# swesterfeld/audiowmark

Hardware: NVIDIA B200
Metric: audio frames/sec embed+detect, 44.1 kHz stereo; decoded-bit match vs ref (higher is better)
Workload: dtype f32

## Files before the change

audiowmark_b200/csrc/awm_capi.cu:

```cuda
#include "awm_kernels.cuh"
#include "awm_speed.cuh"
#include "awm_refine_slide.cuh"
#include "awm_approx_mags.cuh"
#include <vector>
#include <time.h>
#include <string.h>
#include "awm_approx_tc.cuh"
#include "awm_embed_strip.cuh"
#include "awm_viterbi_pair.cuh"

#include <cuda_runtime.h>
#include <dlfcn.h>
#include <algorithm>
#include <map>
#include <thread>
#include <limits.h>
#include <math.h>
#include <stdarg.h>
#include <stdio.h>
#include <string.h>
#include <string>
#include <vector>

using namespace awm;
// ... 49 lines not shown
          }
        if (cur + 1 < chunks.size())
          {
            cur++;
            off = 0;
            continue;
          }
        Chunk c { nullptr, std::max<size_t> (n, size_t (4) << 20) };
        if (cudaMallocHost (reinterpret_cast<void **> (&c.p), c.cap) != cudaSuccess)
          return nullptr;
        chunks.push_back (c);
        cur = chunks.size() - 1;
        off = 0;
      }
  }
  template<class T> T *get (size_t count) { return static_cast<T *> (alloc (std::max<size_t> (count, 1) * sizeof (T))); }
  void release()
  {
    for (auto& c : chunks)
      cudaFreeHost (c.p);
    chunks.clear();
    reset();
  }
};

inline double
wall_now()
{
  timespec ts;
  clock_gettime (CLOCK_MONOTONIC, &ts);
  return double (ts.tv_sec) + 1e-9 * double (ts.tv_nsec);
}

struct SyncTab
{
  DevBuf ent, off, sorted, groups;
  DevBuf masks, masks48, masks64;
  int n_chunks = 0, n_chunks48 = 0, n_chunks64 = 0;
  int n_groups = 0;
  int n_ent = 0, n_bits = 0, total_frames = 0;
  std::vector<awm_sync_entry> h_ent;
  std::vector<int> h_off;
};

struct KeyTab
{
  SyncTab sync[2];
  DevBuf mix, order;
  int n_mix = 0, n_coded = 0, frames_per_bit = 0, fpb = 0;
};

}

struct awm_ctx
{
  int device = 0;
  cudaStream_t stream = nullptr;
  cudaStream_t s_in = nullptr, s_out = nullptr;
  std::string err;
  uint64_t launches = 0;
  int n_sms = 0;
  bool profiling = false;
  struct ProfRec { const char *name; cudaEvent_t e0, e1; double bytes; };
  std::vector<ProfRec> prof;

  DevBuf tw, win, synth;
  DevBuf frame_mod; int embed_fpb = 0;
  KeyTab keys[AWM_MAX_KEYS];

  const float *pcm = nullptr; size_t pcm_frames = 0; int pcm_ch = 0;
  DevBuf pcm_own, pcm16_own;
  struct Prefetch { DevBuf buf, buf16; bool s16 = false; const void *src = nullptr; size_t n_frames = 0; int ch = 0; cudaEvent_t done = nullptr; bool valid = false; };
  Prefetch pref[2];
  int pref_next = 0;
  DevBuf staged, staged16;
  std::vector<cudaEvent_t> stage_done;
  size_t stage_piece = 0, stage_frames = 0, stage_converted = 0;
  int stage_ch = 0;
  bool stage_s16 = false;

  DevBuf dbT, have, q, scores, a_ud, a_cnt, peaks_out, peaks_cnt, a_mags;
  size_t n_scores_dev = 0;
  DevBuf cand_start, cand_noff, r_ud, r_cnt, rvalid, r_ent_ud, r_ent_flag, tw1024;
  DevBuf blk_start, D, raw;
  DevBuf vit_raw, vit_off, vit_types, vit_delta, vit_dec, vit_bits, vit_err, vit_order;
  DevBuf emb_in, emb_out, emb_in16, emb_out16, peaks, snr;

  PinArena pin;

  void *nccl_comm = nullptr;
  int dist_rank = 0, dist_world = 1;
  DevBuf dist_send, dist_recv;
  unsigned char *dist_hsend = nullptr, *dist_hhdr = nullptr;
  size_t dist_hsend_cap = 0;

  struct CoefTab { DevBuf buf; int h = 0; };
  std::map<std::pair<double, int>, CoefTab> coef_cache;
  DevBuf rs_in, rs_out, rs_jobs, pcm_rs;
  const float *saved_pcm = nullptr; size_t saved_frames = 0; int saved_ch = 0; bool pushed = false;
  DevBuf win512, sp_clip, sp_sub, sp_mags, sp_mag_jobs, sp_cmp_jobs, sp_best;
};

namespace {

int
fail (awm_ctx *ctx, const char *fmt, ...)
{
  char buf[512];
  va_list ap;
  va_start (ap, fmt);
  vsnprintf (buf, sizeof (buf), fmt, ap);
  va_end (ap);
  if (ctx)
    ctx->err = buf;
  return 1;
}

#define CK(call) do { cudaError_t e_ = (call); if (e_ != cudaSuccess) return fail (ctx, "%s: %s", #call, cudaGetErrorString (e_)); } while (0)
#define LAUNCH_CHECK(name) do { ctx->launches++; cudaError_t e_ = cudaGetLastError(); if (e_ != cudaSuccess) return fail (ctx, "launch %s: %s", name, cudaGetErrorString (e_)); prof_end (ctx, name); } while (0)
#define PROF(ctx) prof_begin (ctx)

void
prof_begin (awm_ctx *ctx)
{
  if (!ctx->profiling)
    return;
  awm_ctx::ProfRec r;
  r.name = nullptr;
  r.bytes = 0;
  cudaEventCreate (&r.e0);
  cudaEventCreate (&r.e1);
  cudaEventRecord (r.e0, ctx->stream);
  ctx->prof.push_back (r);
}

void
prof_end (awm_ctx *ctx, const char *name)
{
  if (!ctx->profiling || ctx->prof.empty() || ctx->prof.back().name)
    return;
  ctx->prof.back().name = name;
  cudaEventRecord (ctx->prof.back().e1, ctx->stream);
}

void
prof_bytes (awm_ctx *ctx, double bytes)
{
  if (ctx->profiling && !ctx->prof.empty())
    ctx->prof.back().bytes = bytes;
}

bool
is_device_ptr (const void *p)
{
  cudaPointerAttributes a;
  if (cudaPointerGetAttributes (&a, p) != cudaSuccess)
    {
      cudaGetLastError();
      return false;
    }
  return a.type == cudaMemoryTypeDevice || a.type == cudaMemoryTypeManaged;
}

double
window_cos (double x)
{
// ... 21 lines not shown
      weight += w;
    }
  for (int i = 0; i < kFrame; i++)
    win[i] *= 2.0 / weight;
  std::vector<float> synth (3 * kFrame);
  for (int i = 0; i < 3 * kFrame; i++)
    {
      const double overlap = 0.1;
      double norm_pos = (double (i) - kFrame) / kFrame;
      if (norm_pos > 0.5)
        norm_pos = 1 - norm_pos;
      double tri;
      if (norm_pos < -overlap)
        tri = 0;
      else if (norm_pos < overlap)
        tri = 0.5 + norm_pos / (2 * overlap);
      else
        tri = 1;
      synth[i] = (cos (tri * M_PI + M_PI) + 1) * 0.5;
    }
  CK (ctx->tw.reserve (tw.size() * sizeof (float2)));
  CK (ctx->win.reserve (win.size() * sizeof (float)));
  CK (ctx->synth.reserve (synth.size() * sizeof (float)));
  CK (cudaMemcpy (ctx->tw.p, tw.data(), tw.size() * sizeof (float2), cudaMemcpyHostToDevice));
  CK (cudaMemcpy (ctx->win.p, win.data(), win.size() * sizeof (float), cudaMemcpyHostToDevice));
  CK (cudaMemcpy (ctx->synth.p, synth.data(), synth.size() * sizeof (float), cudaMemcpyHostToDevice));
  return 0;
}

template<class K> int
set_smem (awm_ctx *ctx, K kernel, size_t bytes)
{
  static std::map<std::pair<const void *, int>, size_t> done;
  size_t& have = done[{ reinterpret_cast<const void *> (kernel), ctx->device }];
  if (have >= bytes && have)
    return 0;
  CK (cudaFuncSetAttribute (kernel, cudaFuncAttributeMaxDynamicSharedMemorySize, int (bytes)));
  have = bytes;
  return 0;
}

}

void nccl_destroy (void *comm);

extern "C" {

int
awm_create (int device, awm_ctx **out)
{
  if (!out)
    return 1;
  *out = nullptr;
  int n_dev = 0;
  if (cudaGetDeviceCount (&n_dev) != cudaSuccess || n_dev <= 0)
    return 2;
  if (device < 0 || device >= n_dev)
    return 3;
  awm_ctx *ctx = new awm_ctx();
  ctx->device = device;
  if (cudaSetDevice (device) != cudaSuccess || cudaStreamCreateWithFlags (&ctx->stream, cudaStreamNonBlocking) != cudaSuccess)
    {
      delete ctx;
      return 4;
    }
  if (init_tables (ctx))
    {
      fprintf (stderr, "awm_create: %s\n", ctx->err.c_str());
      delete ctx;
      return 5;
    }
  *out = ctx;
  return 0;
}

void
awm_destroy (awm_ctx *ctx)
{
  if (!ctx)
    return;
  cudaSetDevice (ctx->device);
  cudaStreamSynchronize (ctx->stream);
  DevBuf *bufs[] = { &ctx->tw, &ctx->win, &ctx->synth, &ctx->frame_mod, &ctx->pcm_own, &ctx->pcm16_own, &ctx->dbT, &ctx->have, &ctx->q, &ctx->scores, &ctx->a_ud, &ctx->a_cnt, &ctx->peaks_out, &ctx->peaks_cnt, &ctx->a_mags,
                     &ctx->cand_start, &ctx->cand_noff, &ctx->r_ud, &ctx->r_cnt, &ctx->rvalid, &ctx->r_ent_ud, &ctx->r_ent_flag, &ctx->tw1024, &ctx->vit_off, &ctx->blk_start, &ctx->D, &ctx->raw,
                     &ctx->vit_raw, &ctx->vit_types, &ctx->vit_delta, &ctx->vit_dec, &ctx->vit_bits, &ctx->vit_err, &ctx->vit_order,
                     &ctx->emb_in, &ctx->emb_out, &ctx->emb_in16, &ctx->emb_out16, &ctx->peaks, &ctx->snr, &ctx->rs_in, &ctx->rs_out, &ctx->rs_jobs, &ctx->pcm_rs,
                     &ctx->win512, &ctx->sp_clip, &ctx->sp_sub, &ctx->sp_mags, &ctx->sp_mag_jobs, &ctx->sp_cmp_jobs, &ctx->sp_best };
  for (DevBuf *b : bufs)
    b->release();
  ctx->pin.release();
  ctx->dist_send.release();
  ctx->dist_recv.release();
  if (ctx->dist_hsend) cudaFreeHost (ctx->dist_hsend);
  if (ctx->dist_hhdr) cudaFreeHost (ctx->dist_hhdr);
  if (ctx->nccl_comm)
    nccl_destroy (ctx->nccl_comm);
  for (auto& ct : ctx->coef_cache)
    ct.second.buf.release();
  for (auto& pf : ctx->pref)
    {
      pf.buf.release();
      pf.buf16.release();
      if (pf.done)
        cudaEventDestroy (pf.done);
    }
  for (KeyTab& k : ctx->keys)
    {
      for (SyncTab& s : k.sync)
        {
          s.ent.release();
          s.masks.release();
          s.masks48.release();
          s.masks64.release();
          s.off.release();
          s.sorted.release();
          s.groups.release();
        }
      k.mix.release();
      k.order.release();
    }
  for (cudaEvent_t e : ctx->stage_done)
    cudaEventDestroy (e);
  if (ctx->s_in)
    cudaStreamDestroy (ctx->s_in);
  if (ctx->s_out)
    cudaStreamDestroy (ctx->s_out);
  cudaStreamDestroy (ctx->stream);
  delete ctx;
}

const char *
awm_last_error (const awm_ctx *ctx)
{
  return ctx ? ctx->err.c_str() : "no context (is a CUDA device present? there is no CPU fallback)";
}

uint64_t
awm_launch_count (const awm_ctx *ctx)
{
  return ctx ? ctx->launches : 0;
}

void *
awm_stream (awm_ctx *ctx)
{
  return ctx ? (void *) ctx->stream : nullptr;
}

int
awm_synchronize (awm_ctx *ctx)
{
  CK (cudaSetDevice (ctx->device));
  CK (cudaStreamSynchronize (ctx->stream));
  return 0;
}

void *
awm_host_alloc (size_t bytes)
{
  void *p = nullptr;
  if (cudaHostAlloc (&p, bytes ? bytes : 1, cudaHostAllocDefault) != cudaSuccess)
    {
      cudaGetLastError();
      return nullptr;
    }
  return p;
}
// ... 955 lines not shown
  CK (cudaSetDevice (ctx->device));
  const int total = fpb * (mode == AWM_MODE_CLIP ? 2 : 1);
  const double norm_div = water_delta < 0.080 ? water_delta : 0.080;

  const size_t nc = n_scores;
  const int n_bits = t.n_bits;
  CK (ctx->cand_start.reserve (nc * sizeof (long long)));
  CK (ctx->cand_noff.reserve (nc * sizeof (int)));
  CK (ctx->r_ud.reserve (nc * kOffsets * n_bits * 2 * sizeof (float)));
  CK (ctx->r_cnt.reserve (nc * kOffsets * n_bits * sizeof (int)));
  CK (ctx->rvalid.reserve (nc * kOffsets));
  ctx->pin.reset();
  long long *h_start = ctx->pin.get<long long> (nc);
  int *h_noff = ctx->pin.get<int> (nc);
  if (!h_start || !h_noff)
    return fail (ctx, "awm_sync_refine: out of page-locked memory");
  for (size_t c = 0; c < nc; c++)
    {
      const long long idx = (long long) scores[c].index;
      const long long start = std::max<long long> (idx - 256, 0), end = idx + 256;
      h_start[c] = start;
      h_noff[c] = int (std::min<long long> ((end - start) / 8 + 1, kOffsets));
    }
  CK (cudaMemcpyAsync (ctx->cand_start.p, h_start, nc * sizeof (long long), cudaMemcpyHostToDevice, ctx->stream));
  CK (cudaMemcpyAsync (ctx->cand_noff.p, h_noff, nc * sizeof (int), cudaMemcpyHostToDevice, ctx->stream));
  static const bool force_fft = [] { const char *e = getenv ("AWM_REFINE"); return e && !strcmp (e, "fft"); } ();
  const bool used_slide = force < 0 ? (ctx->pcm_ch <= 2 && !force_fft) : (force == 0 && ctx->pcm_ch <= 2);
  if (used_slide)
    {
      if (!ctx->tw1024.p)
        {
          std::vector<float2> tw (1024);
          for (int p = 0; p < 1024; p++)
            {
              const double a = -2.0 * M_PI * double (p) / 1024.0;
              tw[p] = make_float2 (float (cos (a)), float (sin (a)));
            }
          CK (ctx->tw1024.reserve (tw.size() * sizeof (float2)));
          CK (cudaMemcpy (ctx->tw1024.p, tw.data(), tw.size() * sizeof (float2), cudaMemcpyHostToDevice));
        }
      const size_t n_pairs = size_t (nc) * kOffsets * t.n_ent;
      CK (ctx->r_ent_ud.reserve (n_pairs * sizeof (float2)));
      CK (ctx->r_ent_flag.reserve (n_pairs));
      const size_t smem = fft_smem_bytes (kSlideWarps);
      const long long jobs = (long long) nc * t.n_ent;
      const unsigned grid = unsigned ((jobs + kSlideWarps - 1) / kSlideWarps);
      PROF (ctx);
      if (ctx->pcm_ch == 2)
        {
          if (set_smem (ctx, k_refine_slide<2>, smem)) return 1;
          k_refine_slide<2><<<grid, kSlideWarps * 32, smem, ctx->stream>>> (ctx->pcm, (long long) ctx->pcm_frames, ctx->cand_start.as<long long>(), ctx->cand_noff.as<int>(), int (nc),
            t.ent.as<awm_sync_entry>(), t.n_ent, total, (long long) wav_first, (long long) wav_last, ctx->r_ent_ud.as<float2>(), ctx->r_ent_flag.as<unsigned char>(),
            ctx->tw.as<float2>(), ctx->tw1024.as<float2>());
        }
      else
        {
          if (set_smem (ctx, k_refine_slide<1>, smem)) return 1;
          k_refine_slide<1><<<grid, kSlideWarps * 32, smem, ctx->stream>>> (ctx->pcm, (long long) ctx->pcm_frames, ctx->cand_start.as<long long>(), ctx->cand_noff.as<int>(), int (nc),
            t.ent.as<awm_sync_entry>(), t.n_ent, total, (long long) wav_first, (long long) wav_last, ctx->r_ent_ud.as<float2>(), ctx->r_ent_flag.as<unsigned char>(),
            ctx->tw.as<float2>(), ctx->tw1024.as<float2>());
        }
      LAUNCH_CHECK ("k_refine_slide");
      prof_bytes (ctx, double (nc) * double (t.n_ent) * (double (kFrame) + 512.0) * ctx->pcm_ch * sizeof (float));
      const long long n_red = (long long) nc * kOffsets * n_bits;
      PROF (ctx);
      k_refine_reduce<<<unsigned ((n_red + 127) / 128), 128, 0, ctx->stream>>> (ctx->r_ent_ud.as<float2>(), ctx->r_ent_flag.as<unsigned char>(), int (nc), t.n_ent,
        t.off.as<int>(), n_bits, ctx->cand_start.as<long long>(), ctx->cand_noff.as<int>(), (long long) ctx->pcm_frames, total,
        ctx->r_ud.as<float>(), ctx->r_cnt.as<int>(), ctx->rvalid.as<unsigned char>());
      LAUNCH_CHECK ("k_refine_reduce");
    }
  else
    {
      const size_t smem = fft_smem_bytes (kRefineWarps) + kRefineWarps * 96 * sizeof (float);
      if (set_smem (ctx, k_refine, smem)) return 1;
      const long long jobs = (long long) nc * kOffsets * n_bits;
      PROF (ctx);
      k_refine<<<unsigned ((jobs + kRefineWarps - 1) / kRefineWarps), kRefineWarps * 32, smem, ctx->stream>>> (
        ctx->pcm, (long long) ctx->pcm_frames, ctx->pcm_ch, ctx->cand_start.as<long long>(), ctx->cand_noff.as<int>(), int (nc),
        t.ent.as<awm_sync_entry>(), t.off.as<int>(), n_bits, total, (long long) wav_first, (long long) wav_last,
        ctx->r_ud.as<float>(), ctx->r_cnt.as<int>(), ctx->rvalid.as<unsigned char>(), ctx->tw.as<float2>(), ctx->win.as<float>());
      LAUNCH_CHECK ("k_refine");
      prof_bytes (ctx, double (nc) * double (t.n_ent) * (double (kFrame) + 512.0) * ctx->pcm_ch * sizeof (float));
    }
  const size_t n_ud = nc * kOffsets * n_bits * 2, n_cnt = nc * kOffsets * n_bits, n_val = nc * kOffsets;
  float *h_ud = ctx->pin.get<float> (n_ud);
  int *h_cnt = ctx->pin.get<int> (n_cnt);
  unsigned char *h_valid = ctx->pin.get<unsigned char> (n_val);
  if (!h_ud || !h_cnt || !h_valid)
    return fail (ctx, "awm_sync_refine: out of page-locked memory");
  CK (cudaMemcpyAsync (h_ud, ctx->r_ud.p, n_ud * sizeof (float), cudaMemcpyDeviceToHost, ctx->stream));
  CK (cudaMemcpyAsync (h_cnt, ctx->r_cnt.p, n_cnt * sizeof (int), cudaMemcpyDeviceToHost, ctx->stream));
  CK (cudaMemcpyAsync (h_valid, ctx->rvalid.p, n_val, cudaMemcpyDeviceToHost, ctx->stream));
  CK (cudaStreamSynchronize (ctx->stream));
  auto quality_of = [&] (const float *ud, const int *cnt, size_t base) -> double
    {
      double sync_quality = 0;
      int bit_count = 0;
      for (int bit = 0; bit < n_bits; bit++)
        {
          const size_t ob = base * n_bits + bit;
          const float umag = ud[ob * 2], dmag = ud[ob * 2 + 1];
          double raw_bit;
          if (umag == 0 || dmag == 0)
            raw_bit = 0;
          else if (umag < dmag)
            raw_bit = 1 - umag / dmag;
          else
            raw_bit = dmag / umag - 1;
          sync_quality += ((bit & 1) ? raw_bit : -raw_bit) * cnt[ob];
          bit_count += cnt[ob];
        }
      if (bit_count)
        sync_quality /= bit_count;
      return sync_quality / norm_div / 2.9;
    };
  if (q_out)
    {
      for (size_t c = 0; c < nc; c++)
        for (int o = 0; o < kOffsets; o++)
          {
            const bool v = o < h_noff[c] && h_valid[c * kOffsets + o];
            valid_out[c * kOffsets + o] = v ? 1 : 0;
            q_out[c * kOffsets + o] = v ? quality_of (h_ud, h_cnt, c * kOffsets + o) : 0.0;
          }
      return 0;
    }
  if (used_slide)
    {
      constexpr double kVerifyMargin = 1e-3;
      std::vector<long long> p_start;
      std::vector<int> p_noff, p_cand, p_off;
      for (size_t c = 0; c < nc; c++)
        {
          std::vector<std::pair<double, int>> ranked;
          for (int o = 0; o < h_noff[c]; o++)
            if (h_valid[c * kOffsets + o])
              ranked.push_back ({ -fabs (quality_of (h_ud, h_cnt, c * kOffsets + o) - scores[c].local_mean), o });
          std::sort (ranked.begin(), ranked.end());
          size_t keep = 0;
          while (keep < ranked.size() && ranked[keep].first <= ranked[0].first + kVerifyMargin)
            keep++;
          ranked.resize (keep);
          const int o_self = int (((long long) scores[c].index - h_start[c]) / 8);
          if (o_self < h_noff[c] && h_valid[c * kOffsets + o_self]
              && std::find_if (ranked.begin(), ranked.end(), [&] (const std::pair<double, int>& r) { return r.second == o_self; }) == ranked.end())
            ranked.push_back ({ 0.0, o_self });
          std::sort (ranked.begin(), ranked.end(), [] (const std::pair<double, int>& x, const std::pair<double, int>& y) { return x.second < y.second; });
          for (const auto& r : ranked)
            {
              p_start.push_back (h_start[c] + 8LL * r.second);
              p_noff.push_back (1);
              p_cand.push_back (int (c));
              p_off.push_back (r.second);
            }
        }
      const size_t np = p_start.size();
      float *e_ud = ctx->pin.get<float> (np * n_bits * 2);
      int *e_cnt = ctx->pin.get<int> (np * n_bits);
      unsigned char *e_valid = ctx->pin.get<unsigned char> (np);
      long long *e_start = ctx->pin.get<long long> (np);
      if (!e_ud || !e_cnt || !e_valid || !e_start)
        return fail (ctx, "awm_sync_refine: out of page-locked memory");
      std::copy (p_start.begin(), p_start.end(), e_start);
      if (np)
        {
          CK (ctx->cand_start.reserve (np * sizeof (long long)));
          CK (ctx->r_ent_ud.reserve (np * t.n_ent * 2 * kUD * sizeof (float)));
          CK (ctx->r_ud.reserve (np * n_bits * 2 * sizeof (float)));
          CK (ctx->r_cnt.reserve (np * n_bits * sizeof (int)));
          CK (ctx->rvalid.reserve (np));
          CK (cudaMemcpyAsync (ctx->cand_start.p, e_start, np * sizeof (long long), cudaMemcpyHostToDevice, ctx->stream));
          const size_t smem = fft_smem_bytes (kExactWarps) + kExactWarps * 96 * sizeof (float);
          if (set_smem (ctx, k_refine_exact_fft, smem)) return 1;
          const long long jobs = (long long) np * t.n_ent;
          PROF (ctx);
          k_refine_exact_fft<<<unsigned ((jobs + kExactWarps - 1) / kExactWarps), kExactWarps * 32, smem, ctx->stream>>> (
            ctx->pcm, (long long) ctx->pcm_frames, ctx->pcm_ch, ctx->cand_start.as<long long>(), int (np), t.ent.as<awm_sync_entry>(), t.n_ent,
            ctx->r_ent_ud.as<float>(), ctx->tw.as<float2>(), ctx->win.as<float>());
          LAUNCH_CHECK ("k_refine_exact_fft");
          prof_bytes (ctx, double (nc) * double (t.n_ent) * (double (kFrame) + 512.0) * ctx->pcm_ch * sizeof (float));
          PROF (ctx);
          int max_bit_frames = 1;
          for (int b = 0; b < n_bits; b++)
            max_bit_frames = std::max (max_bit_frames, t.h_off[b + 1] - t.h_off[b]);
          const size_t sum_smem = size_t (kExactSumWarps) * max_bit_frames * kUD * sizeof (float);
          if (set_smem (ctx, k_refine_exact_sum, sum_smem)) return 1;
          k_refine_exact_sum<<<unsigned ((np * n_bits * 2 + kExactSumWarps - 1) / kExactSumWarps), kExactSumWarps * 32, sum_smem, ctx->stream>>> (
            ctx->r_ent_ud.as<float>(), ctx->cand_start.as<long long>(), int (np), (long long) ctx->pcm_frames, ctx->pcm_ch, t.ent.as<awm_sync_entry>(), t.n_ent,
            t.off.as<int>(), n_bits, total, (long long) wav_first, (long long) wav_last, max_bit_frames, ctx->r_ud.as<float>(), ctx->r_cnt.as<int>(), ctx->rvalid.as<unsigned char>());
          LAUNCH_CHECK ("k_refine_exact_sum");
          CK (cudaMemcpyAsync (e_ud, ctx->r_ud.p, np * n_bits * 2 * sizeof (float), cudaMemcpyDeviceToHost, ctx->stream));
          CK (cudaMemcpyAsync (e_cnt, ctx->r_cnt.p, np * n_bits * sizeof (int), cudaMemcpyDeviceToHost, ctx->stream));
          CK (cudaMemcpyAsync (e_valid, ctx->rvalid.p, np, cudaMemcpyDeviceToHost, ctx->stream));
          CK (cudaStreamSynchronize (ctx->stream));
        }
      std::vector<double> best_quality (nc);
      std::vector<uint64_t> best_index (nc);
      for (size_t c = 0; c < nc; c++)
        {
          best_quality[c] = scores[c].raw_quality;
          best_index[c] = scores[c].index;
        }
      for (size_t p = 0; p < np; p++)
        if (e_valid[p] && uint64_t (p_start[p]) == scores[p_cand[p]].index)
          best_quality[p_cand[p]] = quality_of (e_ud, e_cnt, p);
      for (size_t p = 0; p < np; p++)
        if (e_valid[p])
          {
            const size_t c = size_t (p_cand[p]);
            const double q = quality_of (e_ud, e_cnt, p);
            if (fabs (q - scores[c].local_mean) > fabs (best_quality[c] - scores[c].local_mean))
              {
                best_quality[c] = q;
                best_index[c] = uint64_t (h_start[c] + 8LL * p_off[p]);
              }
          }
      for (size_t c = 0; c < nc; c++)
        {
          scores[c].index = best_index[c];
          scores[c].raw_quality = best_quality[c];
        }
      return 0;
    }
  for (size_t c = 0; c < nc; c++)
    {
      awm_search_score& sc = scores[c];
      double best_quality = sc.raw_quality;
      uint64_t best_index = sc.index;
      const int o_self = int (((long long) sc.index - h_start[c]) / 8);
      if (o_self < h_noff[c] && h_valid[c * kOffsets + o_self])
        best_quality = quality_of (h_ud, h_cnt, c * kOffsets + o_self);
      for (int o = 0; o < h_noff[c]; o++)
        if (h_valid[c * kOffsets + o])
          {
            const double q = quality_of (h_ud, h_cnt, c * kOffsets + o);
            if (fabs (q - sc.local_mean) > fabs (best_quality - sc.local_mean))
              {
                best_quality = q;
                best_index = uint64_t (h_start[c] + 8LL * o);
              }
          }
      sc.index = best_index;
      sc.raw_quality = best_quality;
    }
  return 0;
}

int
awm_sync_refine (awm_ctx *ctx, int key_slot, int mode, uint64_t wav_first, uint64_t wav_last,
                 double water_delta, awm_search_score *scores, size_t n_scores)
{
  return refine_impl (ctx, key_slot, mode, wav_first, wav_last, water_delta, scores, n_scores, -1, nullptr, nullptr);
}

int
awm_sync_refine_offsets (awm_ctx *ctx, int key_slot, int mode, uint64_t wav_first, uint64_t wav_last, double water_delta,
                         const awm_search_score *scores, size_t n_scores, int exact, double *quality_out, unsigned char *valid_out)
{
  if (!quality_out || !valid_out)
    return fail (ctx, "awm_sync_refine_offsets: bad arguments");
  return refine_impl (ctx, key_slot, mode, wav_first, wav_last, water_delta, const_cast<awm_search_score *> (scores), n_scores, exact ? 1 : 0,
                      quality_out, valid_out);
}

namespace {

struct NcclUniqueId { char internal[128]; };
struct NcclApi
{
  void *lib = nullptr;
  int (*GetUniqueId) (NcclUniqueId *) = nullptr;
  int (*CommInitRank) (void **, int, NcclUniqueId, int) = nullptr;
  int (*AllGather) (const void *, void *, size_t, int, void *, cudaStream_t) = nullptr;
  int (*CommDestroy) (void *) = nullptr;
  const char *(*GetErrorString) (int) = nullptr;
  std::string error;
};

NcclApi&
nccl_api()
{
  static NcclApi api;
  if (api.lib || !api.error.empty())
    return api;
  for (const char *name : { "libnccl.so.2", "libnccl.so" })
    if ((api.lib = dlopen (name, RTLD_NOW | RTLD_GLOBAL)))
      break;
  if (!api.lib)
    {
      api.error = std::string ("cannot load libnccl.so.2: ") + dlerror();
      return api;
    }
  auto sym = [&] (const char *n) { void *p = dlsym (api.lib, n); if (!p) api.error = std::string ("libnccl: missing symbol ") + n; return p; };
  api.GetUniqueId = reinterpret_cast<decltype (api.GetUniqueId)> (sym ("ncclGetUniqueId"));
  api.CommInitRank = reinterpret_cast<decltype (api.CommInitRank)> (sym ("ncclCommInitRank"));
  api.AllGather = reinterpret_cast<decltype (api.AllGather)> (sym ("ncclAllGather"));
  api.CommDestroy = reinterpret_cast<decltype (api.CommDestroy)> (sym ("ncclCommDestroy"));
  api.GetErrorString = reinterpret_cast<decltype (api.GetErrorString)> (sym ("ncclGetErrorString"));
  return api;
}

}

}

void
nccl_destroy (void *comm)
{
  NcclApi& n = nccl_api();
  if (n.CommDestroy)
    n.CommDestroy (comm);
}

extern "C" {

int
awm_dist_unique_id (unsigned char id_out[128])
{
  NcclApi& n = nccl_api();
  if (!n.error.empty() || !id_out)
    return 1;
  NcclUniqueId id;
  if (n.GetUniqueId (&id))
    return 1;
  memcpy (id_out, id.internal, 128);
  return 0;
}
// ... 705 lines not shown
```

audiowmark_b200/csrc/awm_refine_slide.cuh:

```cuda
#pragma once
#include "awm_kernels.cuh"

namespace awm {

constexpr int kSlideWarps = 8;
constexpr int kSlideBins = 3;

template<int C> __global__ void __launch_bounds__ (kSlideWarps * 32, 2)
k_refine_slide (const float *__restrict__ pcm, long long n_frames,
                const long long *__restrict__ cand_start, const int *__restrict__ cand_noff, int n_cand,
                const awm_sync_entry *__restrict__ g_ent, int n_ent, int total_frame_count,
                long long wav_first, long long wav_last,
                float2 *__restrict__ ent_ud , unsigned char *__restrict__ ent_flag,
                const float2 *g_tw, const float2 *__restrict__ tw1024)
{
  extern __shared__ __align__ (16) unsigned char smem[];
  FftSmem s = fft_smem_setup (smem, g_tw, nullptr, kSlideWarps);
  const int lane = threadIdx.x & 31, w = threadIdx.x >> 5;
  const long long job = (long long) blockIdx.x * kSlideWarps + w;
  if (job >= (long long) n_cand * n_ent)
    return;
  const int c = int (job / n_ent), e = int (job % n_ent);
  const awm_sync_entry *en = g_ent + e;
  const long long p0 = cand_start[c] + (long long) en->frame * kFrame;
// ... 132 lines not shown
              const float hr_re = rr_re[b] - 0.5f * (pr_re + qr_re), hr_im = rr_im[b] - 0.5f * (pr_im + qr_im);
              db += db_fast ((hr_re * hr_re + hr_im * hr_im) * 3.814697265625e-06f);
            }
          u = fmaf (db, m_up[b], u);
          d = fmaf (db, m_dn[b], d);
        }
#pragma unroll
      for (int sh = 16; sh > 0; sh >>= 1)
        {
          u += __shfl_xor_sync (0xffffffffu, u, sh);
          d += __shfl_xor_sync (0xffffffffu, d, sh);
        }
      if (lane == 0)
        {
          const long long f_first = start * C, f_last = (start + kFrame) * C;
          const bool counted = !(f_last < wav_first || f_first > wav_last);
          out[(size_t) m * n_ent] = make_float2 (u, d);
          flag[(size_t) m * n_ent] = counted ? 1 : 0;
        }
      if (m + 1 >= n_valid)
        break;
#pragma unroll
      for (int b = 0; b < kSlideBins; b++)
        {
          float tr = rl_re[b], ti = rl_im[b];
#pragma unroll
          for (int j = 0; j < 8; j++)
            {
              tr = fmaf (dl[j], wr[b][j], tr);
              ti = fmaf (dl[j], wi[b][j], ti);
            }
          rl_re[b] = tr * rot_c[b] - ti * rot_s[b];
          rl_im[b] = tr * rot_s[b] + ti * rot_c[b];
          if (C == 2)
            {
              float sr = rr_re[b], si = rr_im[b];
#pragma unroll
              for (int j = 0; j < 8; j++)
                {
                  sr = fmaf (dr[j], wr[b][j], sr);
                  si = fmaf (dr[j], wi[b][j], si);
                }
              rr_re[b] = sr * rot_c[b] - si * rot_s[b];
              rr_im[b] = sr * rot_s[b] + si * rot_c[b];
            }
        }
    }
}

__global__ void
k_refine_reduce (const float2 *__restrict__ ent_ud, const unsigned char *__restrict__ ent_flag, int n_cand, int n_ent,
                 const int *__restrict__ g_bit_off, int n_bits, const long long *__restrict__ cand_start, const int *__restrict__ cand_noff,
                 long long n_frames, int total_frame_count,
                 float *__restrict__ out_ud, int *__restrict__ out_cnt, unsigned char *__restrict__ out_valid)
{
  const long long i = (long long) blockIdx.x * blockDim.x + threadIdx.x;
  if (i >= (long long) n_cand * kOffsets * n_bits)
    return;
  const int c = int (i / (kOffsets * n_bits)), o = int ((i / n_bits) % kOffsets), bit = int (i % n_bits);
  const long long fine = cand_start[c] + 8LL * o;
  const bool valid = o < cand_noff[c] && fine + (long long) total_frame_count * kFrame <= n_frames;
  if (bit == 0)
    out_valid[c * kOffsets + o] = valid ? 1 : 0;
  if (!valid)
    return;
  const float2 *ud = ent_ud + ((size_t) c * kOffsets + o) * n_ent;
  const unsigned char *fl = ent_flag + ((size_t) c * kOffsets + o) * n_ent;
  float umag = 0.f, dmag = 0.f;
  int cnt = 0;
  for (int e = g_bit_off[bit]; e < g_bit_off[bit + 1]; e++)
    if (fl[e])
      {
        const float2 v = ud[e];
        umag += v.x;
        dmag += v.y;
        cnt++;
      }
  const size_t ob = ((size_t) c * kOffsets + o) * n_bits + bit;
  out_ud[ob * 2] = umag;
  out_ud[ob * 2 + 1] = dmag;
  out_cnt[ob] = cnt;
}

}

namespace awm {

constexpr int kExactWarps = 8;

__global__ void __launch_bounds__ (kExactWarps * 32, 2)
k_refine_exact_fft (const float *__restrict__ pcm, long long n_frames, int C, const long long *__restrict__ pair_start, int n_pairs,
                    const awm_sync_entry *__restrict__ g_ent, int n_ent, float *__restrict__ vals ,
                    const float2 *g_tw, const float *g_win)
{
  extern __shared__ __align__ (16) unsigned char smem[];
  FftSmem s = fft_smem_setup (smem, g_tw, g_win, kExactWarps);
  const int lane = threadIdx.x & 31, w = threadIdx.x >> 5;
  float *sband = s.extra + w * 96;
  const long long job = (long long) blockIdx.x * kExactWarps + w;
  if (job >= (long long) n_pairs * n_ent)
    return;
  const int p = int (job / n_ent), e = int (job % n_ent);
  const awm_sync_entry *en = g_ent + e;
  const long long start = pair_start[p] + (long long) en->frame * kFrame;
  float acc[4];
  frame_db_sum (pcm, n_frames, C, start, s, lane, acc);
  bands_to_array (acc, lane, sband, 1);
  __syncwarp();
  float *o = vals + ((size_t) p * n_ent + e) * (2 * kUD);
  if (lane < kUD)
    {
      o[lane] = sband[en->up[lane]];
      o[kUD + lane] = sband[en->down[lane]];
    }
}

constexpr int kExactSumWarps = 4;

__global__ void __launch_bounds__ (kExactSumWarps * 32)
k_refine_exact_sum (const float *__restrict__ vals, const long long *__restrict__ pair_start, int n_pairs, long long n_frames, int C,
                    const awm_sync_entry *__restrict__ g_ent, int n_ent, const int *__restrict__ g_bit_off, int n_bits, int total_frame_count,
                    long long wav_first, long long wav_last, int max_bit_frames,
                    float *__restrict__ out_ud , int *__restrict__ out_cnt, unsigned char *__restrict__ out_valid)
{
  extern __shared__ __align__ (16) unsigned char smem[];
  const int lane = threadIdx.x & 31, w = threadIdx.x >> 5;
  float *stage = reinterpret_cast<float *> (smem) + size_t (w) * max_bit_frames * kUD;
  const int i = blockIdx.x * kExactSumWarps + w;
  if (i >= n_pairs * n_bits * 2)
    return;
  const int p = i / (n_bits * 2), bit = (i / 2) % n_bits, which = i & 1;
  const long long fine = pair_start[p];
  const bool valid = fine + (long long) total_frame_count * kFrame <= n_frames;
  if (bit == 0 && which == 0 && lane == 0)
    out_valid[p] = valid ? 1 : 0;
  if (!valid)
    return;
  const int e0 = g_bit_off[bit], e1 = g_bit_off[bit + 1];
  for (int k = lane; k < (e1 - e0) * kUD; k += 32)
    stage[k] = __ldg (vals + ((size_t) p * n_ent + e0 + k / kUD) * (2 * kUD) + which * kUD + k % kUD);
  __syncwarp();
  if (lane != 0)
    return;
  float mag = 0.f;
  int cnt = 0;
  for (int e = e0; e < e1; e++)
    {
      const long long start = fine + (long long) g_ent[e].frame * kFrame;
      const long long f_first = start * C, f_last = (start + kFrame) * C;
      if (f_last < wav_first || f_first > wav_last)
        continue;
      const float *v = stage + (e - e0) * kUD;
#pragma unroll
      for (int k = 0; k < kUD; k++)
        mag = __fadd_rn (mag, v[k]);
      cnt++;
    }
  out_ud[((size_t) p * n_bits + bit) * 2 + which] = mag;
  if (which == 0)
    out_cnt[(size_t) p * n_bits + bit] = cnt;
}

}
```

Before: 19.61 billion.

## Move sync refine candidate ranking and argmax onto the GPU

```diff
diff --git a/audiowmark_b200/csrc/awm_capi.cu b/audiowmark_b200/csrc/awm_capi.cu
--- a/audiowmark_b200/csrc/awm_capi.cu
+++ b/audiowmark_b200/csrc/awm_capi.cu
@@ -155,6 +155,7 @@
   DevBuf dbT, have, q, scores, a_ud, a_cnt, peaks_out, peaks_cnt, a_mags;
   size_t n_scores_dev = 0;
   DevBuf cand_start, cand_noff, r_ud, r_cnt, rvalid, r_ent_ud, r_ent_flag, tw1024;
+  DevBuf cand_score, pair_start, pair_first, pair_count, pair_n, e_vals, e_ud, e_cnt, e_valid;
   DevBuf blk_start, D, raw;
   DevBuf vit_raw, vit_off, vit_types, vit_delta, vit_dec, vit_bits, vit_err, vit_order;
   DevBuf emb_in, emb_out, emb_in16, emb_out16, peaks, snr;
@@ -342,7 +343,8 @@
   cudaSetDevice (ctx->device);
   cudaStreamSynchronize (ctx->stream);
   DevBuf *bufs[] = { &ctx->tw, &ctx->win, &ctx->synth, &ctx->frame_mod, &ctx->pcm_own, &ctx->pcm16_own, &ctx->dbT, &ctx->have, &ctx->q, &ctx->scores, &ctx->a_ud, &ctx->a_cnt, &ctx->peaks_out, &ctx->peaks_cnt, &ctx->a_mags,
-                     &ctx->cand_start, &ctx->cand_noff, &ctx->r_ud, &ctx->r_cnt, &ctx->rvalid, &ctx->r_ent_ud, &ctx->r_ent_flag, &ctx->tw1024, &ctx->vit_off, &ctx->blk_start, &ctx->D, &ctx->raw,
+                     &ctx->cand_start, &ctx->cand_noff, &ctx->r_ud, &ctx->r_cnt, &ctx->rvalid, &ctx->r_ent_ud, &ctx->r_ent_flag, &ctx->tw1024,
+                     &ctx->cand_score, &ctx->pair_start, &ctx->pair_first, &ctx->pair_count, &ctx->pair_n, &ctx->e_vals, &ctx->e_ud, &ctx->e_cnt, &ctx->e_valid, &ctx->vit_off, &ctx->blk_start, &ctx->D, &ctx->raw,
                      &ctx->vit_raw, &ctx->vit_types, &ctx->vit_delta, &ctx->vit_dec, &ctx->vit_bits, &ctx->vit_err, &ctx->vit_order,
                      &ctx->emb_in, &ctx->emb_out, &ctx->emb_in16, &ctx->emb_out16, &ctx->peaks, &ctx->snr, &ctx->rs_in, &ctx->rs_out, &ctx->rs_jobs, &ctx->pcm_rs,
                      &ctx->win512, &ctx->sp_clip, &ctx->sp_sub, &ctx->sp_mags, &ctx->sp_mag_jobs, &ctx->sp_cmp_jobs, &ctx->sp_best };
@@ -1464,167 +1466,122 @@
       LAUNCH_CHECK ("k_refine");
       prof_bytes (ctx, double (nc) * double (t.n_ent) * (double (kFrame) + 512.0) * ctx->pcm_ch * sizeof (float));
     }
-  const size_t n_ud = nc * kOffsets * n_bits * 2, n_cnt = nc * kOffsets * n_bits, n_val = nc * kOffsets;
-  float *h_ud = ctx->pin.get<float> (n_ud);
-  int *h_cnt = ctx->pin.get<int> (n_cnt);
-  unsigned char *h_valid = ctx->pin.get<unsigned char> (n_val);
-  if (!h_ud || !h_cnt || !h_valid)
-    return fail (ctx, "awm_sync_refine: out of page-locked memory");
-  CK (cudaMemcpyAsync (h_ud, ctx->r_ud.p, n_ud * sizeof (float), cudaMemcpyDeviceToHost, ctx->stream));
-  CK (cudaMemcpyAsync (h_cnt, ctx->r_cnt.p, n_cnt * sizeof (int), cudaMemcpyDeviceToHost, ctx->stream));
-  CK (cudaMemcpyAsync (h_valid, ctx->rvalid.p, n_val, cudaMemcpyDeviceToHost, ctx->stream));
-  CK (cudaStreamSynchronize (ctx->stream));
-  auto quality_of = [&] (const float *ud, const int *cnt, size_t base) -> double
-    {
-      double sync_quality = 0;
-      int bit_count = 0;
-      for (int bit = 0; bit < n_bits; bit++)
-        {
-          const size_t ob = base * n_bits + bit;
-          const float umag = ud[ob * 2], dmag = ud[ob * 2 + 1];
-          double raw_bit;
-          if (umag == 0 || dmag == 0)
-            raw_bit = 0;
-          else if (umag < dmag)
-            raw_bit = 1 - umag / dmag;
-          else
-            raw_bit = dmag / umag - 1;
-          sync_quality += ((bit & 1) ? raw_bit : -raw_bit) * cnt[ob];
-          bit_count += cnt[ob];
-        }
-      if (bit_count)
-        sync_quality /= bit_count;
-      return sync_quality / norm_div / 2.9;
-    };
   if (q_out)
     {
+      const size_t n_ud = nc * kOffsets * n_bits * 2, n_cnt = nc * kOffsets * n_bits, n_val = nc * kOffsets;
+      float *h_ud = ctx->pin.get<float> (n_ud);
+      int *h_cnt = ctx->pin.get<int> (n_cnt);
+      unsigned char *h_valid = ctx->pin.get<unsigned char> (n_val);
+      if (!h_ud || !h_cnt || !h_valid)
+        return fail (ctx, "awm_sync_refine: out of page-locked memory");
+      CK (cudaMemcpyAsync (h_ud, ctx->r_ud.p, n_ud * sizeof (float), cudaMemcpyDeviceToHost, ctx->stream));
+      CK (cudaMemcpyAsync (h_cnt, ctx->r_cnt.p, n_cnt * sizeof (int), cudaMemcpyDeviceToHost, ctx->stream));
+      CK (cudaMemcpyAsync (h_valid, ctx->rvalid.p, n_val, cudaMemcpyDeviceToHost, ctx->stream));
+      CK (cudaStreamSynchronize (ctx->stream));
+      auto quality_of = [&] (size_t base) -> double
+        {
+          double sync_quality = 0;
+          int bit_count = 0;
+          for (int bit = 0; bit < n_bits; bit++)
+            {
+              const size_t ob = base * n_bits + bit;
+              const float umag = h_ud[ob * 2], dmag = h_ud[ob * 2 + 1];
+              double raw_bit;
+              if (umag == 0 || dmag == 0)
+                raw_bit = 0;
+              else if (umag < dmag)
+                raw_bit = 1 - umag / dmag;
+              else
+                raw_bit = dmag / umag - 1;
+              sync_quality += ((bit & 1) ? raw_bit : -raw_bit) * h_cnt[ob];
+              bit_count += h_cnt[ob];
+            }
+          if (bit_count)
+            sync_quality /= bit_count;
+          return sync_quality / norm_div / 2.9;
+        };
       for (size_t c = 0; c < nc; c++)
         for (int o = 0; o < kOffsets; o++)
           {
             const bool v = o < h_noff[c] && h_valid[c * kOffsets + o];
             valid_out[c * kOffsets + o] = v ? 1 : 0;
-            q_out[c * kOffsets + o] = v ? quality_of (h_ud, h_cnt, c * kOffsets + o) : 0.0;
+            q_out[c * kOffsets + o] = v ? quality_of (c * kOffsets + o) : 0.0;
           }
       return 0;
     }
-  if (used_slide)
-    {
-      constexpr double kVerifyMargin = 1e-3;
-      std::vector<long long> p_start;
-      std::vector<int> p_noff, p_cand, p_off;
-      for (size_t c = 0; c < nc; c++)
-        {
-          std::vector<std::pair<double, int>> ranked;
-          for (int o = 0; o < h_noff[c]; o++)
-            if (h_valid[c * kOffsets + o])
-              ranked.push_back ({ -fabs (quality_of (h_ud, h_cnt, c * kOffsets + o) - scores[c].local_mean), o });
-          std::sort (ranked.begin(), ranked.end());
-          size_t keep = 0;
-          while (keep < ranked.size() && ranked[keep].first <= ranked[0].first + kVerifyMargin)
-            keep++;
-          ranked.resize (keep);
-          const int o_self = int (((long long) scores[c].index - h_start[c]) / 8);
-          if (o_self < h_noff[c] && h_valid[c * kOffsets + o_self]
-              && std::find_if (ranked.begin(), ranked.end(), [&] (const std::pair<double, int>& r) { return r.second == o_self; }) == ranked.end())
-            ranked.push_back ({ 0.0, o_self });
-          std::sort (ranked.begin(), ranked.end(), [] (const std::pair<double, int>& x, const std::pair<double, int>& y) { return x.second < y.second; });
-          for (const auto& r : ranked)
-            {
-              p_start.push_back (h_start[c] + 8LL * r.second);
-              p_noff.push_back (1);
-              p_cand.push_back (int (c));
-              p_off.push_back (r.second);
-            }
-        }
-      const size_t np = p_start.size();
-      float *e_ud = ctx->pin.get<float> (np * n_bits * 2);
-      int *e_cnt = ctx->pin.get<int> (np * n_bits);
-      unsigned char *e_valid = ctx->pin.get<unsigned char> (np);
-      long long *e_start = ctx->pin.get<long long> (np);
-      if (!e_ud || !e_cnt || !e_valid || !e_start)
-        return fail (ctx, "awm_sync_refine: out of page-locked memory");
-      std::copy (p_start.begin(), p_start.end(), e_start);
-      if (np)
-        {
-          CK (ctx->cand_start.reserve (np * sizeof (long long)));
-          CK (ctx->r_ent_ud.reserve (np * t.n_ent * 2 * kUD * sizeof (float)));
-          CK (ctx->r_ud.reserve (np * n_bits * 2 * sizeof (float)));
-          CK (ctx->r_cnt.reserve (np * n_bits * sizeof (int)));
-          CK (ctx->rvalid.reserve (np));
-          CK (cudaMemcpyAsync (ctx->cand_start.p, e_start, np * sizeof (long long), cudaMemcpyHostToDevice, ctx->stream));
-          const size_t smem = fft_smem_bytes (kExactWarps) + kExactWarps * 96 * sizeof (float);
-          if (set_smem (ctx, k_refine_exact_fft, smem)) return 1;
-          const long long jobs = (long long) np * t.n_ent;
-          PROF (ctx);
-          k_refine_exact_fft<<<unsigned ((jobs + kExactWarps - 1) / kExactWarps), kExactWarps * 32, smem, ctx->stream>>> (
-            ctx->pcm, (long long) ctx->pcm_frames, ctx->pcm_ch, ctx->cand_start.as<long long>(), int (np), t.ent.as<awm_sync_entry>(), t.n_ent,
-            ctx->r_ent_ud.as<float>(), ctx->tw.as<float2>(), ctx->win.as<float>());
-          LAUNCH_CHECK ("k_refine_exact_fft");
-          prof_bytes (ctx, double (nc) * double (t.n_ent) * (double (kFrame) + 512.0) * ctx->pcm_ch * sizeof (float));
-          PROF (ctx);
-          int max_bit_frames = 1;
-          for (int b = 0; b < n_bits; b++)
-            max_bit_frames = std::max (max_bit_frames, t.h_off[b + 1] - t.h_off[b]);
-          const size_t sum_smem = size_t (kExactSumWarps) * max_bit_frames * kUD * sizeof (float);
-          if (set_smem (ctx, k_refine_exact_sum, sum_smem)) return 1;
-          k_refine_exact_sum<<<unsigned ((np * n_bits * 2 + kExactSumWarps - 1) / kExactSumWarps), kExactSumWarps * 32, sum_smem, ctx->stream>>> (
-            ctx->r_ent_ud.as<float>(), ctx->cand_start.as<long long>(), int (np), (long long) ctx->pcm_frames, ctx->pcm_ch, t.ent.as<awm_sync_entry>(), t.n_ent,
-            t.off.as<int>(), n_bits, total, (long long) wav_first, (long long) wav_last, max_bit_frames, ctx->r_ud.as<float>(), ctx->r_cnt.as<int>(), ctx->rvalid.as<unsigned char>());
-          LAUNCH_CHECK ("k_refine_exact_sum");
-          CK (cudaMemcpyAsync (e_ud, ctx->r_ud.p, np * n_bits * 2 * sizeof (float), cudaMemcpyDeviceToHost, ctx->stream));
-          CK (cudaMemcpyAsync (e_cnt, ctx->r_cnt.p, np * n_bits * sizeof (int), cudaMemcpyDeviceToHost, ctx->stream));
-          CK (cudaMemcpyAsync (e_valid, ctx->rvalid.p, np, cudaMemcpyDeviceToHost, ctx->stream));
-          CK (cudaStreamSynchronize (ctx->stream));
-        }
-      std::vector<double> best_quality (nc);
-      std::vector<uint64_t> best_index (nc);
-      for (size_t c = 0; c < nc; c++)
-        {
-          best_quality[c] = scores[c].raw_quality;
-          best_index[c] = scores[c].index;
-        }
-      for (size_t p = 0; p < np; p++)
-        if (e_valid[p] && uint64_t (p_start[p]) == scores[p_cand[p]].index)
-          best_quality[p_cand[p]] = quality_of (e_ud, e_cnt, p);
-      for (size_t p = 0; p < np; p++)
-        if (e_valid[p])
-          {
-            const size_t c = size_t (p_cand[p]);
-            const double q = quality_of (e_ud, e_cnt, p);
-            if (fabs (q - scores[c].local_mean) > fabs (best_quality[c] - scores[c].local_mean))
-              {
-                best_quality[c] = q;
-                best_index[c] = uint64_t (h_start[c] + 8LL * p_off[p]);
-              }
-          }
-      for (size_t c = 0; c < nc; c++)
-        {
-          scores[c].index = best_index[c];
-          scores[c].raw_quality = best_quality[c];
-        }
+  CK (ctx->cand_score.reserve (nc * sizeof (awm_search_score)));
+  awm_search_score *h_in = ctx->pin.get<awm_search_score> (nc), *h_out = ctx->pin.get<awm_search_score> (nc);
+  unsigned *h_pairs = ctx->pin.get<unsigned> (1);
+  if (!h_in || !h_out || !h_pairs)
+    return fail (ctx, "awm_sync_refine: out of page-locked memory");
+  std::copy (scores, scores + nc, h_in);
+  if (!used_slide)
+    {
+      CK (cudaMemcpyAsync (ctx->cand_score.p, h_in, nc * sizeof (awm_search_score), cudaMemcpyHostToDevice, ctx->stream));
+      PROF (ctx);
+      k_refine_argmax<false><<<unsigned ((nc + 127) / 128), 128, 0, ctx->stream>>> (ctx->cand_score.as<awm_search_score>(), int (nc),
+        nullptr, nullptr, nullptr, nullptr, 0, ctx->cand_start.as<long long>(), ctx->cand_noff.as<int>(),
+        ctx->r_ud.as<float>(), ctx->r_cnt.as<int>(), ctx->rvalid.as<unsigned char>(), n_bits, norm_div);
+      LAUNCH_CHECK ("k_refine_argmax");
+      CK (cudaMemcpyAsync (h_out, ctx->cand_score.p, nc * sizeof (awm_search_score), cudaMemcpyDeviceToHost, ctx->stream));
+      CK (cudaStreamSynchronize (ctx->stream));
+      std::copy (h_out, h_out + nc, scores);
       return 0;
     }
-  for (size_t c = 0; c < nc; c++)
-    {
-      awm_search_score& sc = scores[c];
-      double best_quality = sc.raw_quality;
-      uint64_t best_index = sc.index;
-      const int o_self = int (((long long) sc.index - h_start[c]) / 8);
-      if (o_self < h_noff[c] && h_valid[c * kOffsets + o_self])
-        best_quality = quality_of (h_ud, h_cnt, c * kOffsets + o_self);
-      for (int o = 0; o < h_noff[c]; o++)
-        if (h_valid[c * kOffsets + o])
-          {
-            const double q = quality_of (h_ud, h_cnt, c * kOffsets + o);
-            if (fabs (q - sc.local_mean) > fabs (best_quality - sc.local_mean))
-              {
-                best_quality = q;
-                best_index = uint64_t (h_start[c] + 8LL * o);
-              }
-          }
-      sc.index = best_index;
-      sc.raw_quality = best_quality;
-    }
+  constexpr size_t kPairsPerCand = 4;
+  if (!ctx->n_sms)
+    CK (cudaDeviceGetAttribute (&ctx->n_sms, cudaDevAttrMultiProcessorCount, ctx->device));
+  int max_bit_frames = 1;
+  for (int b = 0; b < n_bits; b++)
+    max_bit_frames = std::max (max_bit_frames, t.h_off[b + 1] - t.h_off[b]);
+  const size_t smem = fft_smem_bytes (kExactWarps) + kExactWarps * 96 * sizeof (float);
+  const size_t sum_smem = size_t (kExactSumWarps) * max_bit_frames * kUD * sizeof (float);
+  if (set_smem (ctx, k_refine_exact_fft, smem) || set_smem (ctx, k_refine_exact_sum, sum_smem))
+    return 1;
+  for (size_t cap = nc * kPairsPerCand;;)
+    {
+      CK (ctx->pair_start.reserve (cap * sizeof (long long)));
+      CK (ctx->pair_first.reserve (nc * sizeof (int)));
+      CK (ctx->pair_count.reserve (nc * sizeof (int)));
+      CK (ctx->pair_n.reserve (sizeof (unsigned)));
+      CK (ctx->e_vals.reserve (cap * t.n_ent * 2 * kUD * sizeof (float)));
+      CK (ctx->e_ud.reserve (cap * n_bits * 2 * sizeof (float)));
+      CK (ctx->e_cnt.reserve (cap * n_bits * sizeof (int)));
+      CK (ctx->e_valid.reserve (cap));
+      CK (cudaMemcpyAsync (ctx->cand_score.p, h_in, nc * sizeof (awm_search_score), cudaMemcpyHostToDevice, ctx->stream));
+      CK (cudaMemsetAsync (ctx->pair_n.p, 0, sizeof (unsigned), ctx->stream));
+      PROF (ctx);
+      k_refine_pick<<<unsigned ((nc * 32 + 127) / 128), 128, 0, ctx->stream>>> (ctx->r_ud.as<float>(), ctx->r_cnt.as<int>(), ctx->rvalid.as<unsigned char>(),
+        ctx->cand_score.as<awm_search_score>(), ctx->cand_start.as<long long>(), ctx->cand_noff.as<int>(), int (nc), n_bits, norm_div,
+        ctx->pair_start.as<long long>(), ctx->pair_first.as<int>(), ctx->pair_count.as<int>(), ctx->pair_n.as<unsigned>(), unsigned (cap));
+      LAUNCH_CHECK ("k_refine_pick");
+      const size_t fft_blocks = std::min<size_t> ((cap * t.n_ent + kExactWarps - 1) / kExactWarps, size_t (ctx->n_sms) * 2);
+      PROF (ctx);
+      k_refine_exact_fft<<<unsigned (fft_blocks), kExactWarps * 32, smem, ctx->stream>>> (
+        ctx->pcm, (long long) ctx->pcm_frames, ctx->pcm_ch, ctx->pair_start.as<long long>(), ctx->pair_n.as<unsigned>(), unsigned (cap),
+        t.ent.as<awm_sync_entry>(), t.n_ent, ctx->e_vals.as<float>(), ctx->tw.as<float2>(), ctx->win.as<float>());
+      LAUNCH_CHECK ("k_refine_exact_fft");
+      prof_bytes (ctx, double (nc) * double (t.n_ent) * (double (kFrame) + 512.0) * ctx->pcm_ch * sizeof (float));
+      const size_t sum_blocks = std::min<size_t> ((cap * n_bits * 2 + kExactSumWarps - 1) / kExactSumWarps, size_t (ctx->n_sms) * 4);
+      PROF (ctx);
+      k_refine_exact_sum<<<unsigned (sum_blocks), kExactSumWarps * 32, sum_smem, ctx->stream>>> (
+        ctx->e_vals.as<float>(), ctx->pair_start.as<long long>(), ctx->pair_n.as<unsigned>(), unsigned (cap), (long long) ctx->pcm_frames, ctx->pcm_ch,
+        t.ent.as<awm_sync_entry>(), t.n_ent, t.off.as<int>(), n_bits, total, (long long) wav_first, (long long) wav_last, max_bit_frames,
+        ctx->e_ud.as<float>(), ctx->e_cnt.as<int>(), ctx->e_valid.as<unsigned char>());
+      LAUNCH_CHECK ("k_refine_exact_sum");
+      PROF (ctx);
+      k_refine_argmax<true><<<unsigned ((nc + 127) / 128), 128, 0, ctx->stream>>> (ctx->cand_score.as<awm_search_score>(), int (nc),
+        ctx->pair_first.as<int>(), ctx->pair_count.as<int>(), ctx->pair_start.as<long long>(), ctx->pair_n.as<unsigned>(), unsigned (cap), nullptr, nullptr,
+        ctx->e_ud.as<float>(), ctx->e_cnt.as<int>(), ctx->e_valid.as<unsigned char>(), n_bits, norm_div);
+      LAUNCH_CHECK ("k_refine_argmax");
+      CK (cudaMemcpyAsync (h_out, ctx->cand_score.p, nc * sizeof (awm_search_score), cudaMemcpyDeviceToHost, ctx->stream));
+      CK (cudaMemcpyAsync (h_pairs, ctx->pair_n.p, sizeof (unsigned), cudaMemcpyDeviceToHost, ctx->stream));
+      CK (cudaStreamSynchronize (ctx->stream));
+      if (*h_pairs <= cap)
+        break;
+      cap = *h_pairs;
+    }
+  std::copy (h_out, h_out + nc, scores);
   return 0;
 }
 
diff --git a/audiowmark_b200/csrc/awm_refine_slide.cuh b/audiowmark_b200/csrc/awm_refine_slide.cuh
--- a/audiowmark_b200/csrc/awm_refine_slide.cuh
+++ b/audiowmark_b200/csrc/awm_refine_slide.cuh
@@ -238,6 +238,138 @@
   out_cnt[ob] = cnt;
 }
 
+__device__ __forceinline__ double
+refine_quality (const float *__restrict__ ud, const int *__restrict__ cnt, int n_bits, double norm_div)
+{
+  double sync_quality = 0;
+  int bit_count = 0;
+  for (int bit = 0; bit < n_bits; bit++)
+    {
+      const float umag = ud[bit * 2], dmag = ud[bit * 2 + 1];
+      float raw_bit;
+      if (umag == 0 || dmag == 0)
+        raw_bit = 0;
+      else if (umag < dmag)
+        raw_bit = __fsub_rn (1.f, __fdiv_rn (umag, dmag));
+      else
+        raw_bit = __fsub_rn (__fdiv_rn (dmag, umag), 1.f);
+      const double signed_bit = (bit & 1) ? double (raw_bit) : -double (raw_bit);
+      sync_quality = __dadd_rn (sync_quality, __dmul_rn (signed_bit, double (cnt[bit])));
+      bit_count += cnt[bit];
+    }
+  if (bit_count)
+    sync_quality = __ddiv_rn (sync_quality, double (bit_count));
+  return __ddiv_rn (__ddiv_rn (sync_quality, norm_div), 2.9);
+}
+
+constexpr double kVerifyMargin = 1e-3;
+
+__global__ void
+k_refine_pick (const float *__restrict__ r_ud, const int *__restrict__ r_cnt, const unsigned char *__restrict__ r_valid,
+               const awm_search_score *__restrict__ scores, const long long *__restrict__ cand_start, const int *__restrict__ cand_noff,
+               int n_cand, int n_bits, double norm_div,
+               long long *__restrict__ pair_start, int *__restrict__ cand_first, int *__restrict__ cand_count, unsigned *__restrict__ n_pairs,
+               unsigned cap)
+{
+  constexpr int kPer = (kOffsets + 31) / 32;
+  const int lane = threadIdx.x & 31;
+  const int c = int (((long long) blockIdx.x * blockDim.x + threadIdx.x) >> 5);
+  if (c >= n_cand)
+    return;
+  const double local_mean = scores[c].local_mean;
+  const long long start = cand_start[c];
+  const int noff = cand_noff[c];
+  const int o_self = int (((long long) scores[c].index - start) / 8);
+  bool valid[kPer];
+  double dist[kPer];
+  double best = -1.0;
+#pragma unroll
+  for (int j = 0; j < kPer; j++)
+    {
+      const int o = lane + 32 * j;
+      const size_t base = (size_t) c * kOffsets + o;
+      valid[j] = o < noff && r_valid[base];
+      dist[j] = valid[j] ? fabs (__dsub_rn (refine_quality (r_ud + base * n_bits * 2, r_cnt + base * n_bits, n_bits, norm_div), local_mean)) : 0.0;
+      if (valid[j])
+        best = fmax (best, dist[j]);
+    }
+#pragma unroll
+  for (int sh = 16; sh > 0; sh >>= 1)
+    best = fmax (best, __shfl_xor_sync (0xffffffffu, best, sh));
+  const double limit = __dadd_rn (-best, kVerifyMargin);
+  unsigned keep[kPer];
+  int total = 0;
+#pragma unroll
+  for (int j = 0; j < kPer; j++)
+    {
+      const int o = lane + 32 * j;
+      keep[j] = __ballot_sync (0xffffffffu, valid[j] && (-dist[j] <= limit || o == o_self));
+      total += __popc (keep[j]);
+    }
+  int first = 0;
+  if (lane == 0)
+    first = total ? int (atomicAdd (n_pairs, unsigned (total))) : 0;
+  first = __shfl_sync (0xffffffffu, first, 0);
+  if (lane == 0)
+    {
+      cand_first[c] = first;
+      cand_count[c] = total;
+    }
+  int at = first;
+#pragma unroll
+  for (int j = 0; j < kPer; j++)
+    {
+      const unsigned slot = unsigned (at + __popc (keep[j] & ((1u << lane) - 1)));
+      if ((keep[j] & (1u << lane)) && slot < cap)
+        pair_start[slot] = start + 8LL * (lane + 32 * j);
+      at += __popc (keep[j]);
+    }
+}
+
+template<bool kList> __global__ void
+k_refine_argmax (awm_search_score *__restrict__ scores, int n_cand, const int *__restrict__ cand_first, const int *__restrict__ cand_count,
+                 const long long *__restrict__ pair_start, const unsigned *__restrict__ n_pairs, unsigned cap,
+                 const long long *__restrict__ cand_start, const int *__restrict__ cand_noff,
+                 const float *__restrict__ ud, const int *__restrict__ cnt, const unsigned char *__restrict__ valid, int n_bits, double norm_div)
+{
+  const int c = blockIdx.x * blockDim.x + threadIdx.x;
+  if (c >= n_cand || (kList && *n_pairs > cap))
+    return;
+  const int first = kList ? cand_first[c] : c * kOffsets;
+  const int count = kList ? cand_count[c] : cand_noff[c];
+  auto start_of = [&] (int p) { return kList ? pair_start[p] : cand_start[c] + 8LL * (p - first); };
+  const double local_mean = scores[c].local_mean;
+  uint64_t best_index = scores[c].index;
+  double best_quality = scores[c].raw_quality;
+  if (kList)
+    {
+      for (int p = first; p < first + count; p++)
+        if (valid[p] && uint64_t (start_of (p)) == best_index)
+          best_quality = refine_quality (ud + (size_t) p * n_bits * 2, cnt + (size_t) p * n_bits, n_bits, norm_div);
+    }
+  else
+    {
+      const int o_self = int (((long long) best_index - cand_start[c]) / 8);
+      if (o_self < count && valid[first + o_self])
+        best_quality = refine_quality (ud + (size_t) (first + o_self) * n_bits * 2, cnt + (size_t) (first + o_self) * n_bits, n_bits, norm_div);
+    }
+  double best_dist = fabs (__dsub_rn (best_quality, local_mean));
+  for (int p = first; p < first + count; p++)
+    if (valid[p])
+      {
+        const double q = refine_quality (ud + (size_t) p * n_bits * 2, cnt + (size_t) p * n_bits, n_bits, norm_div);
+        const double dist = fabs (__dsub_rn (q, local_mean));
+        if (dist > best_dist)
+          {
+            best_quality = q;
+            best_dist = dist;
+            best_index = uint64_t (start_of (p));
+          }
+      }
+  scores[c].index = best_index;
+  scores[c].raw_quality = best_quality;
+}
+
 }
 
 namespace awm {
@@ -245,36 +377,39 @@
 constexpr int kExactWarps = 8;
 
 __global__ void __launch_bounds__ (kExactWarps * 32, 2)
-k_refine_exact_fft (const float *__restrict__ pcm, long long n_frames, int C, const long long *__restrict__ pair_start, int n_pairs,
-                    const awm_sync_entry *__restrict__ g_ent, int n_ent, float *__restrict__ vals ,
+k_refine_exact_fft (const float *__restrict__ pcm, long long n_frames, int C, const long long *__restrict__ pair_start, const unsigned *__restrict__ n_pairs,
+                    unsigned cap, const awm_sync_entry *__restrict__ g_ent, int n_ent, float *__restrict__ vals ,
                     const float2 *g_tw, const float *g_win)
 {
   extern __shared__ __align__ (16) unsigned char smem[];
   FftSmem s = fft_smem_setup (smem, g_tw, g_win, kExactWarps);
   const int lane = threadIdx.x & 31, w = threadIdx.x >> 5;
   float *sband = s.extra + w * 96;
-  const long long job = (long long) blockIdx.x * kExactWarps + w;
-  if (job >= (long long) n_pairs * n_ent)
-    return;
-  const int p = int (job / n_ent), e = int (job % n_ent);
-  const awm_sync_entry *en = g_ent + e;
-  const long long start = pair_start[p] + (long long) en->frame * kFrame;
-  float acc[4];
-  frame_db_sum (pcm, n_frames, C, start, s, lane, acc);
-  bands_to_array (acc, lane, sband, 1);
-  __syncwarp();
-  float *o = vals + ((size_t) p * n_ent + e) * (2 * kUD);
-  if (lane < kUD)
-    {
-      o[lane] = sband[en->up[lane]];
-      o[kUD + lane] = sband[en->down[lane]];
+  const long long jobs = (long long) min (*n_pairs, cap) * n_ent;
+  for (long long job = (long long) blockIdx.x * kExactWarps + w; job < jobs; job += (long long) gridDim.x * kExactWarps)
+    {
+      const int p = int (job / n_ent), e = int (job % n_ent);
+      const awm_sync_entry *en = g_ent + e;
+      const long long start = pair_start[p] + (long long) en->frame * kFrame;
+      float acc[4];
+      frame_db_sum (pcm, n_frames, C, start, s, lane, acc);
+      bands_to_array (acc, lane, sband, 1);
+      __syncwarp();
+      float *o = vals + ((size_t) p * n_ent + e) * (2 * kUD);
+      if (lane < kUD)
+        {
+          o[lane] = sband[en->up[lane]];
+          o[kUD + lane] = sband[en->down[lane]];
+        }
+      __syncwarp();
     }
 }
 
 constexpr int kExactSumWarps = 4;
 
 __global__ void __launch_bounds__ (kExactSumWarps * 32)
-k_refine_exact_sum (const float *__restrict__ vals, const long long *__restrict__ pair_start, int n_pairs, long long n_frames, int C,
+k_refine_exact_sum (const float *__restrict__ vals, const long long *__restrict__ pair_start, const unsigned *__restrict__ n_pairs, unsigned cap,
+                    long long n_frames, int C,
                     const awm_sync_entry *__restrict__ g_ent, int n_ent, const int *__restrict__ g_bit_off, int n_bits, int total_frame_count,
                     long long wav_first, long long wav_last, int max_bit_frames,
                     float *__restrict__ out_ud , int *__restrict__ out_cnt, unsigned char *__restrict__ out_valid)
@@ -282,39 +417,42 @@
   extern __shared__ __align__ (16) unsigned char smem[];
   const int lane = threadIdx.x & 31, w = threadIdx.x >> 5;
   float *stage = reinterpret_cast<float *> (smem) + size_t (w) * max_bit_frames * kUD;
-  const int i = blockIdx.x * kExactSumWarps + w;
-  if (i >= n_pairs * n_bits * 2)
-    return;
-  const int p = i / (n_bits * 2), bit = (i / 2) % n_bits, which = i & 1;
-  const long long fine = pair_start[p];
-  const bool valid = fine + (long long) total_frame_count * kFrame <= n_frames;
-  if (bit == 0 && which == 0 && lane == 0)
-    out_valid[p] = valid ? 1 : 0;
-  if (!valid)
-    return;
-  const int e0 = g_bit_off[bit], e1 = g_bit_off[bit + 1];
-  for (int k = lane; k < (e1 - e0) * kUD; k += 32)
-    stage[k] = __ldg (vals + ((size_t) p * n_ent + e0 + k / kUD) * (2 * kUD) + which * kUD + k % kUD);
-  __syncwarp();
-  if (lane != 0)
-    return;
-  float mag = 0.f;
-  int cnt = 0;
-  for (int e = e0; e < e1; e++)
-    {
-      const long long start = fine + (long long) g_ent[e].frame * kFrame;
-      const long long f_first = start * C, f_last = (start + kFrame) * C;
-      if (f_last < wav_first || f_first > wav_last)
+  const int n_items = int (min (*n_pairs, cap)) * n_bits * 2;
+  for (int i = blockIdx.x * kExactSumWarps + w; i < n_items; i += gridDim.x * kExactSumWarps)
+    {
+      const int p = i / (n_bits * 2), bit = (i / 2) % n_bits, which = i & 1;
+      const long long fine = pair_start[p];
+      const bool valid = fine + (long long) total_frame_count * kFrame <= n_frames;
+      if (bit == 0 && which == 0 && lane == 0)
+        out_valid[p] = valid ? 1 : 0;
+      if (!valid)
         continue;
-      const float *v = stage + (e - e0) * kUD;
-#pragma unroll
-      for (int k = 0; k < kUD; k++)
-        mag = __fadd_rn (mag, v[k]);
-      cnt++;
-    }
-  out_ud[((size_t) p * n_bits + bit) * 2 + which] = mag;
-  if (which == 0)
-    out_cnt[(size_t) p * n_bits + bit] = cnt;
-}
-
-}
+      const int e0 = g_bit_off[bit], e1 = g_bit_off[bit + 1];
+      for (int k = lane; k < (e1 - e0) * kUD; k += 32)
+        stage[k] = __ldg (vals + ((size_t) p * n_ent + e0 + k / kUD) * (2 * kUD) + which * kUD + k % kUD);
+      __syncwarp();
+      if (lane == 0)
+        {
+          float mag = 0.f;
+          int cnt = 0;
+          for (int e = e0; e < e1; e++)
+            {
+              const long long start = fine + (long long) g_ent[e].frame * kFrame;
+              const long long f_first = start * C, f_last = (start + kFrame) * C;
+              if (f_last < wav_first || f_first > wav_last)
+                continue;
+              const float *v = stage + (e - e0) * kUD;
+#pragma unroll
+              for (int k = 0; k < kUD; k++)
+                mag = __fadd_rn (mag, v[k]);
+              cnt++;
+            }
+          out_ud[((size_t) p * n_bits + bit) * 2 + which] = mag;
+          if (which == 0)
+            out_cnt[(size_t) p * n_bits + bit] = cnt;
+        }
+      __syncwarp();
+    }
+}
+
+}
```

Measured after the change: 20.08 billion, median of 6. +2.4%, better.
